# aokomoriuta/ConjugateGradient

Measured on AMD Instinct MI355X. Metric: CG iterations/sec (7-pt Poisson 512^3); SpMV achieved HBM GB/s in roofline, higher is better.
Workload: dtype f64

## Files before the change

### conjugategradient_amd/csrc/common.hpp

```cpp
#pragma once
#include <hip/hip_runtime.h>
#include <cstddef>
#include <cstdint>
#include <cstdio>
#include <cstdarg>
#include <cstring>
#include <cmath>
#include <atomic>
#include <mutex>
#include <string>
#include <type_traits>
#include <vector>

#pragma GCC visibility push(default)
#include "../../include/MgcgGpu.h"
#pragma GCC visibility pop

namespace mgcg {

constexpr int kWave = 64;
constexpr int kBlock = 256;
constexpr int kNumXcd = 8;
constexpr int kNumCu = 256;
constexpr int kMaxGrid = kNumCu * 8;
// ... 379 lines not shown
struct SpmvConfig { int kernel = 0; int rowsPerBlock = 64; int flags = 0; int gridBlocks = 0; int periodRows = 0; int tileRows = 0; int tilePlanes = 0;
                    int maxRow = 0;  };

int launch_spmv(hipStream_t s, int epilogue, const SpmvArgs& a, const SpmvConfig& cfg);
inline bool spmv_takes_rowtile(const SpmvArgs& a, const SpmvConfig& cfg)
{
    int kernel = cfg.kernel;
    if (kernel == 0) kernel = spmv_auto_kernel(a.rowCount > 0 ? (double)a.elementsCount / (double)a.rowCount : 0.0);
    return kernel == 10 && (((uintptr_t)a.elements & 15) == 0) && (((uintptr_t)a.columnIndeces & 15) == 0) && a.elementsCount >= 8 && a.rowCount > 0;
}
int launch_spmv_rowtile(hipStream_t s, int epilogue, const SpmvArgs& a, int periodRows, int gridReq, int maxRow = 0, bool ntWindow = false,
                        int gapAtTile = 0, int gapSkipTiles = 0);
int spmv_period(MgcgSparse* h, const int* rowOffsets, const int* columnIndeces, long long rows, long long rowBase, int* maxRow = nullptr, long long* meanDistance = nullptr);
void launch_matrix_shape(hipStream_t s, const int* rowOffsets, const int* columnIndeces, long long rows, long long row, long long rowBase, int* out2);
int launch_spmv_rows(hipStream_t s, int epilogue, const SpmvArgs& a, const DcsrView* m, int gridReq, int periodRows = 0);
bool dcsr_build(hipStream_t s, const double* elements, const int* rowOffsets, const int* columnIndeces,
                long long rows, long long nnz, long long rowBase, DcsrMatrix* out);
bool pattern_build(hipStream_t s, const double* elements, const int* rowOffsets, const int* columnIndeces,
                   long long rows, long long nnz, long long rowBase, DcsrMatrix* out);
bool tiled_build(hipStream_t s, const double* elements, const int* rowOffsets, const int* columnIndeces,
                 long long rows, long long nnz, long long rowBase, long long columns, DcsrMatrix* out);
int launch_spmv_tiled(hipStream_t s, int epilogue, const SpmvArgs& a, const DcsrView& m);
bool exclusive_scan(hipStream_t s, int* data, long long n);
bool pb_build(hipStream_t s, const double* elements, const int* rowOffsets, const int* columnIndeces,
              long long rows, long long nnz, long long columns, long long meanDistance, DcsrMatrix* out);
int launch_spmv_pb(hipStream_t s, int epilogue, const SpmvArgs& a, const DcsrView& m);
const DcsrMatrix* dcsr_lookup(MgcgSparse* h, const double* elements, const int* rowOffsets, const int* columnIndeces,
                              long long rows, long long nnz, long long rowBase, long long columns = 0,
                              long long autoMeanDistance = -1,
                              bool trustRegistry = false);
const DcsrMatrix* dcsr_lookup_op(MgcgSparse* h, const SpmvArgs& a, long long rowBase);
bool vector_owned(const void* p, size_t bytes);
void vector_registry_add(const void* p, size_t bytes);
void vector_registry_remove(const void* p);
unsigned long long csr_checksum(hipStream_t s, const double* elements, const int* rowOffsets, const int* columnIndeces, long long rows, long long nnz, unsigned long long* scratch);
void analysis_note_write(const void* p, size_t bytes);
int launch_spmv_auto(hipStream_t s, int epilogue, const SpmvArgs& a, const SpmvConfig& cfg, const DcsrMatrix* dc);
int launch_spmv_range(hipStream_t s, int epilogue, const SpmvArgs& a, const SpmvConfig& cfg, const DcsrMatrix* dc,
                      long long r0, long long r1, double* partials, int maxGrid);

int launch_spmv_two_ranges(hipStream_t s, int epilogue, const SpmvArgs& a, const SpmvConfig& cfg, const DcsrMatrix* dc,
                           long long i0, long long i1, double* partials, int maxGrid);

void launch_axpy(hipStream_t s, double* y, const double* x, long long n, double alpha);
void launch_scal(hipStream_t s, double* x, double alpha, long long n);
void launch_xpay(hipStream_t s, double* y, const double* x, long long n, double beta);
// ... 189 lines not shown
    default:                 converged = (it >= f.minIt) && (it <= f.maxIt) && (d.res < f.tol); break;
    }
    d.status = MGCG_OK;
    d.stop = converged;
    if (!d.stop && it >= f.minIt && it > f.maxIt) { d.stop = true; d.status = MGCG_MAXIT_EXCEEDED; }
    if (!d.stop && !(d.res == d.res && fabs(d.res) <= 1.79e308)) { d.stop = true; d.status = MGCG_NONFINITE; }
    return d;
}
void launch_reduce_to(hipStream_t s, const double* partials, int n, double* dst, const int* done);
void launch_reduce2_to(hipStream_t s, const double* pA, int nA, double* dstA, const double* pB, int nB, double* dstB, const int* done);
void launch_finalize(hipStream_t s, const double* partials, const double* partialsInf, int n, bool reduceFirst, const FinalizeArgs& f);
void launch_finalize_precond(hipStream_t s, const double* partials, int n, bool reduceFirst, CgScalars* sc);
void launch_init_scalars(hipStream_t s, const double* partials, const double* partialsZ, int n, bool reduceFirst, CgScalars* sc, HostMirror* mirror);

void launch_jacobi_first(hipStream_t s, long long n, double omega, const double* dinv, int dinvUniform, double dinvScalar, const double* b, double* x, const int* done);
void launch_uniform_check(hipStream_t s, const double* v, long long n, int* flag);
void launch_restrict(hipStream_t s, int nx, int ny, int nz, const double* r, double* bc, const int* done);
void launch_prolong_add(hipStream_t s, int nx, int ny, int nz, double* x, const double* e, const int* done);
void launch_prolong_linear_add(hipStream_t s, int nx, int ny, int nz, int z0, int z1, double* x, const double* eFull, const int* done);
void launch_restrict_linear(hipStream_t s, int nx, int ny, int nz, int z0, int z1, const double* rFull, double* bc, const int* done);
void launch_prolong_scaled(hipStream_t s, int nx, int ny, int nz, double* x, const double* b, double inner, double outer, const double* e, const int* done);
void launch_extract_dinv(hipStream_t s, const double* elements, const int* rowOffsets, const int* columnIndeces,
                         long long n, long long rowBase, double* dinv);
void launch_galerkin(hipStream_t s, int nx, int ny, int nz, int zBegin, int zEnd, const double* elements, const int* rowOffsets, const int* columnIndeces,
                     double sigma, const int* rowOffsetsC, int* countsC, double* elementsC, int* columnIndecesC, int* errFlag);
void launch_poisson(hipStream_t s, int nx, int ny, int nz, int zBegin, int zEnd, double* elements, int* rowOffsets, int* columnIndeces);
void launch_rebase(hipStream_t s, int* rowOffsets, long long n, int base);
long long poisson_nnz_host(int nx, int ny, int nz, int zBegin, int zEnd);
void launch_minmax_int(hipStream_t s, const int* v, long long n, int* out2 );
void launch_halo_rows(hipStream_t s, const int* rowOffsets, const int* columnIndeces, long long n, long long offset, int* out2 );

void launch_amg_restrict(hipStream_t s, long long nc, const int* aggOffsets, const int* members, const double* r, double* bc, const int* done);
void launch_amg_prolong_add(hipStream_t s, long long n, const int* agg, double* x, const double* e, const int* done);
void launch_amg_check_diagonal(hipStream_t s, const double* elements, const int* rowOffsets, const int* columnIndeces, long long n, int* badRow);
void launch_amg_row_max(hipStream_t s, const double* elements, const int* rowOffsets, const int* columnIndeces, long long n, double* rowMax);
void launch_amg_match_round(hipStream_t s, const double* elements, const int* rowOffsets, const int* columnIndeces, long long n, double theta,
                            const double* rowMax, int* match, int* pick, int* flags2);
void launch_amg_galerkin_count(hipStream_t s, long long nc, const int* aggOffsets, const int* members, const int* rowOffsets, const int* columnIndeces,
                               const int* agg, const int* expandOffsets, int* scratch, int* counts);
void launch_amg_galerkin_fill(hipStream_t s, long long nc, const int* aggOffsets, const int* members, const double* elements, const int* rowOffsets,
                              const int* columnIndeces, const int* agg, const int* expandOffsets, const int* scratch, const int* rowOffsetsC, double sigma,
                              double* elementsC, int* columnIndecesC);
void launch_amg_gather_values(hipStream_t s, long long m, const int* source, const double* elements, double* out);

constexpr int kTransposeShortMax = 32;
constexpr int kTransposeLdsMax = 4096;
void launch_transpose_check_offsets(hipStream_t s, const int* rowOffsets, long long rows, int* status3);
void launch_transpose_count(hipStream_t s, const int* rowOffsets, const int* columnIndeces, long long rows, long long columns, long long nnz, int* counts, int* badRow);
// ... 47 lines not shown
```

### conjugategradient_amd/csrc/kernels_mg.hip

```cpp
#include "common.hpp"

namespace mgcg {

static inline int grid1(long long n)
{
    long long b = (n + kBlock - 1) / kBlock;
    if (b > kMaxGrid) b = kMaxGrid;
    if (b < 1) b = 1;
    return (int)b;
}

typedef double d2mg __attribute__((ext_vector_type(2)));

template <bool UNIFORM>
__global__ __launch_bounds__(kBlock) void jacobi_first_kernel(long long n, double omega, const double* __restrict__ dinv, double dscalar,
                                                              const double* __restrict__ b, double* __restrict__ x, const int* done)
{
    if (done != nullptr && *done != 0) return;
    const bool wide = ((((uintptr_t)b) | ((uintptr_t)x) | ((uintptr_t)dinv)) & 15) == 0;
    if (wide) {
        const long long n2 = n >> 1;
        const long long per = ((n2 + gridDim.x - 1) / gridDim.x + (kBlock - 1)) & ~(long long)(kBlock - 1);
        long long end = per * (blockIdx.x + 1);
        end = end < n2 ? end : n2;
// ... 323 lines not shown
        return;
    }
    const long long NC = (long long)(nx > 1 ? nx / 2 : 1) * (ny > 1 ? ny / 2 : 1) * ((z1 - z0) / (nz > 1 ? 2 : 1));
    hipLaunchKernelGGL(restrict_linear_kernel, dim3(grid1(NC)), dim3(kBlock), 0, s, nx, ny, nz, z0, z1, rFull, bc, done);
}

__global__ __launch_bounds__(kBlock) void extract_dinv_kernel(const double* __restrict__ elements, const int* __restrict__ rowOffsets,
                                                              const int* __restrict__ columnIndeces, long long n, long long rowBase, double* __restrict__ dinv)
{
    const long long stride = (long long)gridDim.x * kBlock;
    for (long long i = (long long)blockIdx.x * kBlock + threadIdx.x; i < n; i += stride) {
        double d = 0.0;
        for (int k = rowOffsets[i]; k < rowOffsets[i + 1]; ++k)
            if (columnIndeces[k] == rowBase + i) { d = elements[k]; break; }
        dinv[i] = 1.0 / d;
    }
}
void launch_extract_dinv(hipStream_t s, const double* elements, const int* rowOffsets, const int* columnIndeces,
                         long long n, long long rowBase, double* dinv)
{
    hipLaunchKernelGGL(extract_dinv_kernel, dim3(grid1(n)), dim3(kBlock), 0, s, elements, rowOffsets, columnIndeces, n, rowBase, dinv);
}

__global__ __launch_bounds__(kBlock) void galerkin_kernel(int nx, int ny, int nz, int zBegin, int zEnd,
                                                          const double* __restrict__ elements, const int* __restrict__ rowOffsets,
                                                          const int* __restrict__ columnIndeces, double sigma, const int* __restrict__ rowOffsetsC,
                                                          int* __restrict__ countsC, double* __restrict__ elementsC, int* __restrict__ columnIndecesC, int* errFlag)
{
    const int cx = nx > 1 ? 2 : 1, cy = ny > 1 ? 2 : 1, cz = nz > 1 ? 2 : 1;
    const int NX = nx / cx, NY = ny / cy;
    const int ZL = (zEnd - zBegin) / cz;
    const int Z0 = zBegin / cz;
    const long long NC = (long long)NX * NY * ZL;
    const long long sxy = (long long)nx * ny;
    const long long stride = (long long)gridDim.x * kBlock;
    for (long long I = (long long)blockIdx.x * kBlock + threadIdx.x; I < NC; I += stride) {
        const int X = (int)(I % NX), Y = (int)((I / NX) % NY), Zl = (int)(I / ((long long)NX * NY));
        const int Z = Z0 + Zl;
        double acc[27];
        unsigned touched = 0u;
#pragma unroll
        for (int q = 0; q < 27; ++q) acc[q] = 0.0;
        for (int dz = 0; dz < cz; ++dz)
            for (int dy = 0; dy < cy; ++dy)
                for (int dx = 0; dx < cx; ++dx) {
                    const long long i = ((long long)(Zl * cz + dz) * ny + (Y * cy + dy)) * nx + (X * cx + dx);
                    for (int k = rowOffsets[i]; k < rowOffsets[i + 1]; ++k) {
                        const long long j = columnIndeces[k];
                        const int jx = (int)(j % nx), jy = (int)((j / nx) % ny), jz = (int)(j / sxy);
                        const int ox = jx / cx - X, oy = jy / cy - Y, oz = jz / cz - Z;
                        if (ox < -1 || ox > 1 || oy < -1 || oy > 1 || oz < -1 || oz > 1) { *errFlag = 1; continue; }
                        const int q = (oz + 1) * 9 + (oy + 1) * 3 + (ox + 1);
                        const double v = elements[k];
#pragma unroll
                        for (int t = 0; t < 27; ++t) if (t == q) acc[t] += v;
                        touched |= 1u << q;
                    }
                }
        if (elementsC == nullptr) { countsC[I] = __popc(touched); continue; }
        int kout = rowOffsetsC[I];
#pragma unroll
        for (int q = 0; q < 27; ++q) {
            if (!(touched & (1u << q))) continue;
            const int ox = q % 3 - 1, oy = (q / 3) % 3 - 1, oz = q / 9 - 1;
            elementsC[kout] = sigma * acc[q];
            columnIndecesC[kout] = (int)(((long long)(Z + oz) * NY + (Y + oy)) * NX + (X + ox));
            ++kout;
        }
    }
}
void launch_galerkin(hipStream_t s, int nx, int ny, int nz, int zBegin, int zEnd, const double* elements, const int* rowOffsets, const int* columnIndeces,
                     double sigma, const int* rowOffsetsC, int* countsC, double* elementsC, int* columnIndecesC, int* errFlag)
{
    const long long NC = (long long)(nx > 1 ? nx / 2 : 1) * (ny > 1 ? ny / 2 : 1) * (nz > 1 ? (zEnd - zBegin) / 2 : 1);
    hipLaunchKernelGGL(galerkin_kernel, dim3(grid1(NC)), dim3(kBlock), 0, s, nx, ny, nz, zBegin, zEnd, elements, rowOffsets, columnIndeces,
                       sigma, rowOffsetsC, countsC, elementsC, columnIndecesC, errFlag);
}

__device__ __host__ inline long long poisson_row_offset(long long i, int nx, int ny, int nz)
{
    const long long sxy = (long long)nx * ny;
    const int x = (int)(i % nx), y = (int)((i / nx) % ny), z = (int)(i / sxy);
    const long long L = i / nx;
    long long missing = 0;
    missing += L + (x > 0 ? 1 : 0);
    missing += L;
    missing += (long long)z * nx + (y > 0 ? nx : x);
    missing += (long long)z * nx + (y == ny - 1 ? x : 0);
    if (nz > 1) {
        missing += (z > 0) ? sxy : ((long long)y * nx + x);
        missing += (z == nz - 1) ? ((long long)y * nx + x) : 0;
        return 7 * i - missing;
    }
    return 5 * i - missing;
}

__global__ __launch_bounds__(kBlock) void poisson_kernel(int nx, int ny, int nz, int zBegin, int zEnd,
                                                         double* __restrict__ elements, int* __restrict__ rowOffsets, int* __restrict__ columnIndeces)
{
// ... 103 lines not shown
```

### conjugategradient_amd/csrc/kernels_tiled.hip

```cpp
#include "common.hpp"
#include <algorithm>

namespace mgcg {

constexpr int kScanBlock = 256;
constexpr int kScanPer = 8;

__global__ __launch_bounds__(kBlock) void tiled_count_kernel(const int* __restrict__ rowOffsets, const int* __restrict__ columnIndeces,
                                                             long long rows, long long rowBase, int tileWidth, int nTiles,
                                                             int* __restrict__ counts, unsigned long long* stats )
{
    const long long stride = (long long)gridDim.x * kBlock;
    unsigned long long far = 0, unsorted = 0;
    for (long long i = (long long)blockIdx.x * kBlock + threadIdx.x; i < rows; i += stride) {
        const int s = rowOffsets[i], e = rowOffsets[i + 1];
        int prev = -1, tile = -1, run = 0;
        for (int k = s; k < e; ++k) {
            const int c = columnIndeces[k];
            if (c <= prev) unsorted = 1;
            prev = c;
            const long long d = (long long)c - (rowBase + i);
            far += (unsigned long long)((d < 0 ? -d : d) >> 10);
            const int t = c / tileWidth;
            if (t != tile) { if (tile >= 0 && tile < nTiles) counts[(long long)tile * rows + i] = run; tile = t; run = 0; }
// ... 5 lines not shown
    if (unsorted) atomicAdd(&stats[0], 1ull);
}

__global__ __launch_bounds__(kScanBlock) void scan_local_kernel(int* __restrict__ data, long long n, int* __restrict__ blockTotals)
{
    __shared__ int s_sum[kScanBlock];
    const long long base = ((long long)blockIdx.x * kScanBlock + threadIdx.x) * kScanPer;
    int v[kScanPer], total = 0;
#pragma unroll
    for (int j = 0; j < kScanPer; ++j) { v[j] = (base + j < n) ? data[base + j] : 0; total += v[j]; }
    s_sum[threadIdx.x] = total;
    __syncthreads();
    for (int off = 1; off < kScanBlock; off <<= 1) {
        const int add = threadIdx.x >= off ? s_sum[threadIdx.x - off] : 0;
        __syncthreads();
        s_sum[threadIdx.x] += add;
        __syncthreads();
    }
    int run = s_sum[threadIdx.x] - total;
#pragma unroll
    for (int j = 0; j < kScanPer; ++j) { if (base + j < n) data[base + j] = run; run += v[j]; }
    if (threadIdx.x == kScanBlock - 1) blockTotals[blockIdx.x] = s_sum[kScanBlock - 1];
}
__global__ __launch_bounds__(kScanBlock) void scan_totals_kernel(int* __restrict__ blockTotals, int nBlocks)
{
    __shared__ int s_sum[kScanBlock];
    __shared__ int s_carry;
    if (threadIdx.x == 0) s_carry = 0;
    __syncthreads();
    for (int base = 0; base < nBlocks; base += kScanBlock) {
        const int i = base + threadIdx.x;
        const int v = i < nBlocks ? blockTotals[i] : 0;
        s_sum[threadIdx.x] = v;
        __syncthreads();
        for (int off = 1; off < kScanBlock; off <<= 1) {
            const int add = threadIdx.x >= off ? s_sum[threadIdx.x - off] : 0;
            __syncthreads();
            s_sum[threadIdx.x] += add;
            __syncthreads();
        }
        if (i < nBlocks) blockTotals[i] = s_carry + s_sum[threadIdx.x] - v;
        __syncthreads();
        if (threadIdx.x == kScanBlock - 1) s_carry += s_sum[kScanBlock - 1];
        __syncthreads();
    }
}
__global__ __launch_bounds__(kScanBlock) void scan_add_kernel(int* __restrict__ data, long long n, const int* __restrict__ blockTotals)
{
    const long long base = ((long long)blockIdx.x * kScanBlock + threadIdx.x) * kScanPer;
    const int add = blockTotals[blockIdx.x];
#pragma unroll
    for (int j = 0; j < kScanPer; ++j) if (base + j < n) data[base + j] += add;
}

__global__ __launch_bounds__(kBlock) void tiled_zero_kernel(double* __restrict__ y, long long n, const int* __restrict__ doneFlag)
{
    if (doneFlag != nullptr && *doneFlag != 0) return;
    const long long stride = (long long)gridDim.x * kBlock;
    for (long long i = (long long)blockIdx.x * kBlock + threadIdx.x; i < n; i += stride) y[i] = 0.0;
}
static int grid_rows(long long n)
{
    const long long blocks = (n + kBlock - 1) / kBlock;
    return (int)(blocks < 1 ? 1 : (blocks > kMaxGrid ? kMaxGrid : blocks));
}

__global__ __launch_bounds__(kBlock) void tiled_scatter_kernel(const double* __restrict__ elements, const int* __restrict__ rowOffsets,
                                                               const int* __restrict__ columnIndeces, long long rows, int tileWidth,
// ... 179 lines not shown
        hipLaunchKernelGGL(spmv_tile_pass_kernel<false>, g, dim3(kBlock), 0, s, a.x, a.y, m.tileVals, m.tileCols, m.tileRowIds, kb, ke, a.doneFlag);
    }
    if (EPI == EPI_AXPBY && a.alpha == 1.0) return 0;
    const int grid = grid_rows(a.rowCount);
    hipLaunchKernelGGL((tiled_epilogue_kernel<EPI>), dim3(grid), dim3(kBlock), 0, s, a);
    return grid;
}

int launch_spmv_tiled(hipStream_t s, int epilogue, const SpmvArgs& a, const DcsrView& m)
{
    if (a.rowCount <= 0) return 0;
    switch (epilogue) {
    case EPI_AXPBY:        return launch_tiled_epi<EPI_AXPBY>(s, a, m);
    case EPI_DOT:          return launch_tiled_epi<EPI_DOT>(s, a, m);
    case EPI_RESIDUAL:     return launch_tiled_epi<EPI_RESIDUAL>(s, a, m);
    case EPI_RESIDUAL_DOT: return launch_tiled_epi<EPI_RESIDUAL_DOT>(s, a, m);
    case EPI_JACOBI:       return launch_tiled_epi<EPI_JACOBI>(s, a, m);
    case EPI_JACOBI_DOT:   return launch_tiled_epi<EPI_JACOBI_DOT>(s, a, m);
    }
    set_error("column-tiled SpMV: epilogue %d is not implemented (the Chebyshev step multiplies through the CSR kernels)", epilogue);
    return 0;
}

bool exclusive_scan(hipStream_t s, int* data, long long n)
{
    const long long perBlock = (long long)kScanBlock * kScanPer;
    const long long nBlocks = (n + perBlock - 1) / perBlock;
    if (nBlocks > 0x7fffffffLL) { set_error("tiled analysis: too many scan blocks"); return false; }
    int* totals = nullptr;
    if (!MGCG_HIP(hipMalloc((void**)&totals, sizeof(int) * (size_t)nBlocks))) return false;
    hipLaunchKernelGGL(scan_local_kernel, dim3((unsigned)nBlocks), dim3(kScanBlock), 0, s, data, n, totals);
    hipLaunchKernelGGL(scan_totals_kernel, dim3(1), dim3(kScanBlock), 0, s, totals, (int)nBlocks);
    hipLaunchKernelGGL(scan_add_kernel, dim3((unsigned)nBlocks), dim3(kScanBlock), 0, s, data, n, totals);
    const bool ok = MGCG_HIP(hipGetLastError()) && MGCG_HIP(hipStreamSynchronize(s));
    (void)hipFree(totals);
    return ok;
}

bool tiled_build(hipStream_t s, const double* elements, const int* rowOffsets, const int* columnIndeces,
                 long long rows, long long nnz, long long rowBase, long long columns, DcsrMatrix* out)
{
    int tileShift = 19;
    long long tileCols = 365LL * 1024;
    { const int v = tuning().tileShift.load(std::memory_order_relaxed); if (v >= 8 && v <= 26) { tileShift = v; tileCols = 1LL << v; } }
    const int nTiles = (int)((columns + tileCols - 1) / tileCols);
    const int tileWidth = nTiles > 0 ? (int)((columns + nTiles - 1) / nTiles) : (int)tileCols;
    if (rows <= 0 || nnz <= 0 || nTiles < 4 || nTiles > 256) return true;
    const long long cells = (long long)nTiles * rows;
    {
        size_t freeB = 0, totalB = 0;
        if (hipMemGetInfo(&freeB, &totalB) != hipSuccess) { (void)hipGetLastError(); return true; }
        const double need = 4.0 * (double)(cells + 1) + 16.0 * (double)nnz;
        if (cells + 1 > 0x7fffffffLL * 4LL || need > 0.5 * (double)freeB) return true;
    }
    int* counts = nullptr; unsigned long long* stats = nullptr;
    double* tv = nullptr; int* tc = nullptr; int* tr = nullptr;
// ... 88 lines not shown
```

### conjugategradient_amd/csrc/solver.hip

```cpp
#include "common.hpp"
#include <algorithm>
#include <chrono>
#include <functional>

namespace mgcg {

struct MgLevel {
    int nx = 0, ny = 0, nz = 0;
    int z0 = 0, z1 = 0;
    long long n = 0, nnz = 0;
    long long nGlobal = 0, offset = 0;
    double* elements = nullptr; int* rowOffsets = nullptr; int* columnIndeces = nullptr;
    bool ownsMatrix = false;
    double* dinv = nullptr;
    bool dinvUniform = false; double dinvScalar = 0.0;
    double *xa = nullptr, *xb = nullptr;
    double *b = nullptr, *r = nullptr;
    SpmvConfig cfg;
    const DcsrMatrix* dcsr = nullptr;
    HaloPlan* halo = nullptr;
    HaloPlan* transferHalo = nullptr;
    int minJ = 0, maxJ = -1;
    bool overlap = false;
    long long interior0 = 0, interior1 = 0;
// ... 2003 lines not shown
                        int elementsCount, int nx, int ny, int nz, int zBegin, int zEnd,
                        int levels, double omega, int nu, int nuCoarse, double sigma)
{
    DeviceState* d = device_state();
    if (!d) return nullptr;
    const long long nGlobal0 = (long long)nx * ny * nz;
    const int nranks = MgcgCommSize(comm);
    const long long nLocal0 = (long long)nx * ny * (zEnd - zBegin);
    bool pre = true;
    if (!cublas || !cusparse || !elementsVector || !rowOffsetsVector || !columnIndecesVector) { set_error("MgSetup: null argument"); pre = false; }
    if (pre && (nx < 1 || ny < 1 || nz < 1 || levels < 1 || nu < 1 || nuCoarse < 1 || nGlobal0 > 0x7fffffffLL || zBegin < 0 || zEnd > nz || zBegin >= zEnd)) { set_error("MgSetup: bad parameters"); pre = false; }
    if (pre && (rowOffsetsVector->size < nLocal0 + 1 || elementsVector->size < elementsCount || columnIndecesVector->size < elementsCount)) { set_error("MgSetup: matrix vectors too small"); pre = false; }
    if (pre && nranks > 1 && (nz % nranks != 0 || (zEnd - zBegin) != nz / nranks || zBegin != MgcgCommRank(comm) * (nz / nranks))) {
        set_error("MgSetup: with several ranks the grid must be split into equal z-slabs in rank order"); pre = false;
    }
    if (!comm_agree(comm, pre, "MgSetup")) return nullptr;
    hipStream_t s = d->stream;
    MgcgMg* mg = new MgcgMg();
    mg->omega = omega; mg->nu = nu; mg->nuCoarse = nuCoarse; mg->sigma = sigma; mg->stream = s; mg->cfg = cfg_of(cusparse);
    mg->cfg.kernel = 0;
    mg->comm = comm; mg->nranks = nranks; mg->multi = comm_multi(comm);
    mg->haloOnSide = tuning().haloStream.load(std::memory_order_relaxed) != 0;
    const bool multi = mg->multi;
    int* dErr = nullptr;
    int* dmm = nullptr;
    bool ok = MGCG_HIP(hipMalloc((void**)&dErr, sizeof(int))) && MGCG_HIP(hipMemsetAsync(dErr, 0, sizeof(int), s)) && MGCG_HIP(hipMalloc((void**)&dmm, 2 * sizeof(int)));
    auto coarse_matrix = [&](MgLevel& L, const MgLevel& F) -> bool {
        L.ownsMatrix = true;
        int* counts = nullptr;
        bool good = MGCG_HIP(hipMalloc((void**)&L.rowOffsets, sizeof(int) * (size_t)(L.n + 1))) && MGCG_HIP(hipMalloc((void**)&counts, sizeof(int) * (size_t)(L.n > 0 ? L.n : 1)));
        std::vector<int> h((size_t)L.n + 1);
        int err = 0;
        if (good) {
            launch_galerkin(s, F.nx, F.ny, F.nz, F.z0, F.z1, F.elements, F.rowOffsets, F.columnIndeces, sigma, nullptr, counts, nullptr, nullptr, dErr);
            good = MGCG_HIP(hipMemcpyAsync(h.data() + 1, counts, sizeof(int) * (size_t)L.n, hipMemcpyDeviceToHost, s)) &&
                   MGCG_HIP(hipMemcpyAsync(&err, dErr, sizeof(int), hipMemcpyDeviceToHost, s)) && MGCG_HIP(hipStreamSynchronize(s));
        }
        if (counts) (void)hipFree(counts);
        if (!good) return false;
        if (err) { set_error("MgSetup: matrix is not a 27-point-neighbourhood operator on the %dx%dx%d grid", F.nx, F.ny, F.nz); return false; }
        h[0] = 0;
        long long run = 0;
        for (long long i = 1; i <= L.n; ++i) { run += h[(size_t)i]; h[(size_t)i] = (int)run; }
        L.nnz = run;
        good = MGCG_HIP(hipMemcpyAsync(L.rowOffsets, h.data(), sizeof(int) * (size_t)(L.n + 1), hipMemcpyHostToDevice, s)) &&
               MGCG_HIP(hipMalloc((void**)&L.elements, sizeof(double) * (size_t)(L.nnz > 0 ? L.nnz : 1))) &&
               MGCG_HIP(hipMalloc((void**)&L.columnIndeces, sizeof(int) * (size_t)(L.nnz > 0 ? L.nnz : 1)));
        if (good) launch_galerkin(s, F.nx, F.ny, F.nz, F.z0, F.z1, F.elements, F.rowOffsets, F.columnIndeces, sigma, L.rowOffsets, nullptr, L.elements, L.columnIndeces, dErr);
        return MGCG_HIP(hipStreamSynchronize(s)) && good;
    };
    bool agreedToLeave = false;
    for (int l = 0; ok && l < levels; ++l) {
        MgLevel L;
        if (l == 0) {
            L.nx = nx; L.ny = ny; L.nz = nz; L.z0 = zBegin; L.z1 = zEnd; L.nnz = elementsCount;
            L.elements = elementsVector->data; L.rowOffsets = rowOffsetsVector->data; L.columnIndeces = columnIndecesVector->data;
        } else {
            const MgLevel& F = mg->lv[l - 1];
            if ((F.nx > 1 && F.nx % 2) || (F.ny > 1 && F.ny % 2) || (F.nz > 1 && F.nz % 2)) break;
            if (F.nx == 1 && F.ny == 1 && F.nz == 1) break;
            if (F.nz > 1 && ((F.z0 % 2) || (F.z1 % 2))) break;
            if (nranks > 1 && F.nz == 1) break;
            L.nx = F.nx > 1 ? F.nx / 2 : 1; L.ny = F.ny > 1 ? F.ny / 2 : 1; L.nz = F.nz > 1 ? F.nz / 2 : 1;
            L.z0 = F.nz > 1 ? F.z0 / 2 : 0; L.z1 = F.nz > 1 ? F.z1 / 2 : 1;
        }
        L.nGlobal = (long long)L.nx * L.ny * L.nz;
        L.n = (long long)L.nx * L.ny * (L.z1 - L.z0);
        L.offset = (long long)L.nx * L.ny * L.z0;
        if (l > 0) ok = ok && coarse_matrix(L, mg->lv[l - 1]);
        ok = ok && MGCG_HIP(hipMalloc((void**)&L.dinv, sizeof(double) * (size_t)L.n));
        ok = ok && MGCG_HIP(hipMalloc((void**)&L.xa, sizeof(double) * (size_t)L.nGlobal));
        ok = ok && MGCG_HIP(hipMalloc((void**)&L.r, sizeof(double) * (size_t)L.n));
        if (l > 0 || multi) ok = ok && MGCG_HIP(hipMalloc((void**)&L.xb, sizeof(double) * (size_t)L.nGlobal));
        if (l > 0) ok = ok && MGCG_HIP(hipMalloc((void**)&L.b, sizeof(double) * (size_t)L.n));
        if (ok && multi) {
            ok = ok && MGCG_HIP(hipMemsetAsync(L.xa, 0, sizeof(double) * (size_t)L.nGlobal, s)) && MGCG_HIP(hipMemsetAsync(L.xb, 0, sizeof(double) * (size_t)L.nGlobal, s));
        }
        if (ok) launch_extract_dinv(s, L.elements, L.rowOffsets, L.columnIndeces, L.n, L.offset, L.dinv);
        if (ok && L.n > 0) {
            int differs = 1;
            ok = MGCG_HIP(hipMemsetAsync(dmm, 0, sizeof(int), s));
            if (ok) launch_uniform_check(s, L.dinv, L.n, dmm);
            ok = ok && MGCG_HIP(hipMemcpyAsync(&differs, dmm, sizeof(int), hipMemcpyDeviceToHost, s)) &&
                 MGCG_HIP(hipMemcpyAsync(&L.dinvScalar, L.dinv, sizeof(double), hipMemcpyDeviceToHost, s)) && MGCG_HIP(hipStreamSynchronize(s));
            L.dinvUniform = ok && differs == 0;
        }
        if (ok) L.dcsr = dcsr_lookup(cusparse, L.elements, L.rowOffsets, L.columnIndeces, L.n, L.nnz, L.offset);
        L.cfg = mg->cfg;
        if (ok && L.nnz >= 8) (void)spmv_period(cusparse, L.rowOffsets, L.columnIndeces, L.n, L.offset, &L.cfg.maxRow);
        L.cfg.periodRows = (L.nz > 1) ? L.nx * L.ny : 0;
        if (ok && multi) {
            int init[2] = { 0x7fffffff, (int)0x80000000 }, out[2] = { 0, -1 };
            ok = ok && MGCG_HIP(hipMemcpyAsync(dmm, init, sizeof(init), hipMemcpyHostToDevice, s));
            if (ok && L.nnz > 0) launch_minmax_int(s, L.columnIndeces, L.nnz, dmm);
            ok = ok && MGCG_HIP(hipMemcpyAsync(out, dmm, sizeof(out), hipMemcpyDeviceToHost, s));
            ok = ok && MGCG_HIP(hipStreamSynchronize(s));
            L.minJ = out[0]; L.maxJ = out[1];
        }
        if (multi) {
            ok = comm_agree(comm, ok, "MgSetup");
            if (ok) { L.halo = halo_plan_create(comm, L.nGlobal, L.offset, L.n, L.minJ, L.maxJ); ok = comm_agree(comm, L.halo != nullptr, "MgSetup"); }
            agreedToLeave = !ok;
            ok = ok && plan_overlap(s, comm, mg->multi, L.rowOffsets, L.columnIndeces, L.n, L.offset, &L.overlap, &L.interior0, &L.interior1, cublas->ws.devInts + 6, L.halo, L.xa, L.nGlobal);
        }
        mg->lv.push_back(L);
        if (!ok) break;
        mg->levels = (int)mg->lv.size();
    }
    ok = ok && MGCG_HIP(hipStreamSynchronize(s));
    if (dErr) (void)hipFree(dErr);
    if (dmm) (void)hipFree(dmm);
    bool wantDeep = ok && multi && nu == 1 && mg->levels >= 2 && tuning().deepHalo.load(std::memory_order_relaxed) != 0;
    bool foldsEverywhere = true;
    for (int l = 1; wantDeep && l < mg->levels; ++l) {
        const MgLevel& L = mg->lv[(size_t)l];
        const int d = (l == mg->levels - 1) ? nuCoarse : 2;
        if (L.nz <= 1 || (L.z1 - L.z0) < d || (L.z0 & 1) || ((L.z1 - L.z0) & 1)) wantDeep = false;
    }
    if (multi && (agreedToLeave || !comm_agree(comm, ok, "MgSetup"))) { MgDestroy(mg); return nullptr; }
    for (int l = 1; ok && wantDeep && l < mg->levels; ++l) {
        MgLevel& L = mg->lv[(size_t)l];
        const long long plane = (long long)L.nx * L.ny;
        const int d = (l == mg->levels - 1) ? nuCoarse : 2;
        L.deep = d;
        L.extZ0 = L.z0 - d < 0 ? 0 : L.z0 - d;
        L.extZ1 = L.z1 + d > L.nz ? L.nz : L.z1 + d;
        L.extBase = (long long)L.extZ0 * plane; L.extRows = (long long)(L.extZ1 - L.extZ0) * plane;
        const long long edge = (long long)d * plane;
        std::vector<int> ro((size_t)L.n + 1);
        bool lok = MGCG_HIP(hipMemcpyAsync(ro.data(), L.rowOffsets, sizeof(int) * (size_t)(L.n + 1), hipMemcpyDeviceToHost, s)) && MGCG_HIP(hipStreamSynchronize(s));
        auto pack = [&](long long r0, long long r1, std::vector<double>& out) {
            out.clear();
            if (!lok || r1 <= r0) return;
// ... 1450 lines not shown
```

Baseline: 275.6.

## Tile Galerkin coarsening in LDS, scan row offsets on device, fuse dinv extraction

Rewrites the Galerkin coarse-operator kernel to stage row offsets, column indices and values for a tile of 64 coarse rows in shared memory. It replaces integer division with magic-number reciprocals and splits the 27 stencil slots across four lanes per coarse row. The host-side prefix sum and its round trip are replaced by a device exclusive scan. The coarse diagonal inverse and its uniformity check are computed inside the fill kernel, which removes the separate extract and check passes and several stream syncs. All of this is MG setup work, so the timed CG/SpMV iteration throughput is unlikely to change.

```diff
diff --git a/conjugategradient_amd/csrc/common.hpp b/conjugategradient_amd/csrc/common.hpp
--- a/conjugategradient_amd/csrc/common.hpp
+++ b/conjugategradient_amd/csrc/common.hpp
@@ -425,6 +425,8 @@
                  long long rows, long long nnz, long long rowBase, long long columns, DcsrMatrix* out);
 int launch_spmv_tiled(hipStream_t s, int epilogue, const SpmvArgs& a, const DcsrView& m);
 bool exclusive_scan(hipStream_t s, int* data, long long n);
+long long exclusive_scan_blocks(long long n);
+void exclusive_scan_enqueue(hipStream_t s, int* data, long long n, int* totals, int* totalOut);
 bool pb_build(hipStream_t s, const double* elements, const int* rowOffsets, const int* columnIndeces,
               long long rows, long long nnz, long long columns, long long meanDistance, DcsrMatrix* out);
 int launch_spmv_pb(hipStream_t s, int epilogue, const SpmvArgs& a, const DcsrView& m);
@@ -660,8 +662,15 @@
 void launch_prolong_scaled(hipStream_t s, int nx, int ny, int nz, double* x, const double* b, double inner, double outer, const double* e, const int* done);
 void launch_extract_dinv(hipStream_t s, const double* elements, const int* rowOffsets, const int* columnIndeces,
                          long long n, long long rowBase, double* dinv);
+struct MgSetupRecord {
+    int nnz;
+    int err;
+    unsigned long long dinvHi;
+    unsigned long long dinvLo;
+    double dinvFirst;
+};
 void launch_galerkin(hipStream_t s, int nx, int ny, int nz, int zBegin, int zEnd, const double* elements, const int* rowOffsets, const int* columnIndeces,
-                     double sigma, const int* rowOffsetsC, int* countsC, double* elementsC, int* columnIndecesC, int* errFlag);
+                     long long nnzF, double sigma, const int* rowOffsetsC, int* countsC, double* elementsC, int* columnIndecesC, double* dinvC, MgSetupRecord* rec);
 void launch_poisson(hipStream_t s, int nx, int ny, int nz, int zBegin, int zEnd, double* elements, int* rowOffsets, int* columnIndeces);
 void launch_rebase(hipStream_t s, int* rowOffsets, long long n, int base);
 long long poisson_nnz_host(int nx, int ny, int nz, int zBegin, int zEnd);
diff --git a/conjugategradient_amd/csrc/kernels_mg.hip b/conjugategradient_amd/csrc/kernels_mg.hip
--- a/conjugategradient_amd/csrc/kernels_mg.hip
+++ b/conjugategradient_amd/csrc/kernels_mg.hip
@@ -369,59 +369,234 @@
     hipLaunchKernelGGL(extract_dinv_kernel, dim3(grid1(n)), dim3(kBlock), 0, s, elements, rowOffsets, columnIndeces, n, rowBase, dinv);
 }
 
+typedef int i4mg __attribute__((ext_vector_type(4)));
+constexpr int kGalTile = 64;
+constexpr int kGalRuns = 4;
+constexpr int kGalCap = kGalRuns * 2 * kGalTile * 7 + 8 * kGalRuns;
+static_assert(kBlock == 4 * kGalTile, "four lanes per coarse row of a tile");
+
+struct GalDiv { unsigned long long m; int shift; };
+__device__ __forceinline__ GalDiv gal_div(unsigned d)
+{
+    const int l = d > 1u ? 32 - __clz((int)(d - 1u)) : 0;
+    return { ((1ull << (31 + l)) + d - 1u) / d, 31 + l };
+}
+__device__ __forceinline__ unsigned gal_quot(unsigned n, GalDiv g) { return (unsigned)(((unsigned long long)n * g.m) >> g.shift); }
+
+struct GalGrid { unsigned nx, sxy; GalDiv byLine, byPlane; int sx, sy, sz; };
+__device__ __forceinline__ int gal_slot(const GalGrid& g, int col, int X, int Y, int Z)
+{
+    if (col < 0) return -1;
+    const unsigned j = (unsigned)col;
+    const unsigned jz = gal_quot(j, g.byPlane), rem = j - jz * g.sxy, jy = gal_quot(rem, g.byLine), jx = rem - jy * g.nx;
+    const int ox = (int)(jx >> g.sx) - X, oy = (int)(jy >> g.sy) - Y, oz = (int)(jz >> g.sz) - Z;
+    if (ox < -1 || ox > 1 || oy < -1 || oy > 1 || oz < -1 || oz > 1) return -1;
+    return (oz + 1) * 9 + (oy + 1) * 3 + (ox + 1);
+}
+
+template <bool FILL>
 __global__ __launch_bounds__(kBlock) void galerkin_kernel(int nx, int ny, int nz, int zBegin, int zEnd,
                                                           const double* __restrict__ elements, const int* __restrict__ rowOffsets,
-                                                          const int* __restrict__ columnIndeces, double sigma, const int* __restrict__ rowOffsetsC,
-                                                          int* __restrict__ countsC, double* __restrict__ elementsC, int* __restrict__ columnIndecesC, int* errFlag)
-{
+                                                          const int* __restrict__ columnIndeces, long long nnzF, double sigma,
+                                                          const int* __restrict__ rowOffsetsC, int* __restrict__ countsC, double* __restrict__ elementsC,
+                                                          int* __restrict__ columnIndecesC, double* __restrict__ dinvC, MgSetupRecord* rec)
+{
+    __shared__ int s_ro[kGalRuns][2 * kGalTile + 1];
+    __shared__ __attribute__((aligned(16))) int s_col[kGalCap];
+    __shared__ __attribute__((aligned(16))) double s_val[FILL ? kGalCap : 2];
+    __shared__ unsigned s_touched[kGalTile];
+    __shared__ unsigned long long s_hi, s_lo;
     const int cx = nx > 1 ? 2 : 1, cy = ny > 1 ? 2 : 1, cz = nz > 1 ? 2 : 1;
     const int NX = nx / cx, NY = ny / cy;
     const int ZL = (zEnd - zBegin) / cz;
     const int Z0 = zBegin / cz;
-    const long long NC = (long long)NX * NY * ZL;
-    const long long sxy = (long long)nx * ny;
-    const long long stride = (long long)gridDim.x * kBlock;
-    for (long long I = (long long)blockIdx.x * kBlock + threadIdx.x; I < NC; I += stride) {
-        const int X = (int)(I % NX), Y = (int)((I / NX) % NY), Zl = (int)(I / ((long long)NX * NY));
+    const int runs = cy * cz;
+    const int tilesX = (NX + kGalTile - 1) / kGalTile;
+    const long long nTiles = (long long)tilesX * NY * ZL;
+    GalGrid grid;
+    grid.nx = (unsigned)nx; grid.sxy = (unsigned)nx * (unsigned)ny;
+    grid.byLine = gal_div(grid.nx); grid.byPlane = gal_div(grid.sxy);
+    grid.sx = cx - 1; grid.sy = cy - 1; grid.sz = cz - 1;
+    const bool aligned = ((((uintptr_t)elements) | ((uintptr_t)columnIndeces)) & 15) == 0;
+    const int mine = (int)threadIdx.x & (kGalTile - 1), part = (int)threadIdx.x / kGalTile;
+    unsigned long long hi = 0ull, lo = 0ull;
+    if (threadIdx.x == 0) { s_hi = 0ull; s_lo = 0ull; }
+    for (long long tile = blockIdx.x; tile < nTiles; tile += gridDim.x) {
+        const int X0 = (int)(tile % tilesX) * kGalTile;
+        const long long line = tile / tilesX;
+        const int Y = (int)(line % NY), Zl = (int)(line / NY);
         const int Z = Z0 + Zl;
-        double acc[27];
-        unsigned touched = 0u;
-#pragma unroll
-        for (int q = 0; q < 27; ++q) acc[q] = 0.0;
-        for (int dz = 0; dz < cz; ++dz)
-            for (int dy = 0; dy < cy; ++dy)
+        const long long I0 = ((long long)Zl * NY + Y) * NX + X0;
+        const int rowsC = NX - X0 < kGalTile ? NX - X0 : kGalTile;
+        const int rowsF = rowsC * cx;
+        for (int t = threadIdx.x; t < runs * (rowsF + 1); t += kBlock) {
+            const int r = t / (rowsF + 1), f = t - r * (rowsF + 1);
+            const int dz = r / cy, dy = r - dz * cy;
+            const long long i0 = ((long long)(Zl * cz + dz) * ny + (Y * cy + dy)) * nx + X0 * cx;
+            s_ro[r][f] = rowOffsets[i0 + f];
+        }
+        if (!FILL && threadIdx.x < kGalTile) s_touched[threadIdx.x] = 0u;
+        __syncthreads();
+        int a0[kGalRuns], a1[kGalRuns], base[kGalRuns];
+        int total = 0;
+        bool sane = true;
+#pragma unroll
+        for (int r = 0; r < kGalRuns; ++r) {
+            a0[r] = 0; a1[r] = 0; base[r] = total;
+            if (r < runs) {
+                a0[r] = s_ro[r][0] & ~3;
+                a1[r] = (s_ro[r][rowsF] + 3) & ~3;
+                sane = sane && s_ro[r][0] >= 0 && a1[r] >= a0[r] && a1[r] - a0[r] <= kGalCap;
+                total += a1[r] - a0[r];
+            }
+        }
+        const bool parked = aligned && sane && total <= kGalCap;
+        if (parked) {
+#pragma unroll
+            for (int r = 0; r < kGalRuns; ++r) {
+                const int groups = (a1[r] - a0[r]) >> 2;
+                for (int g = threadIdx.x; g < groups; g += kBlock) {
+                    const long long k = (long long)a0[r] + 4 * g;
+                    const int at = base[r] + 4 * g;
+                    if (k + 4 <= nnzF) {
+                        *(i4mg*)&s_col[at] = *(const i4mg*)&columnIndeces[k];
+                        if (FILL) {
+                            *(d2mg*)&s_val[at] = *(const d2mg*)&elements[k];
+                            *(d2mg*)&s_val[at + 2] = *(const d2mg*)&elements[k + 2];
+                        }
+                    } else {
+                        for (int j = 0; j < 4; ++j)
+                            if (k + j < nnzF) { s_col[at + j] = columnIndeces[k + j]; if (FILL) s_val[at + j] = elements[k + j]; }
+                    }
+                }
+            }
+            __syncthreads();
+            for (int t = threadIdx.x; t < runs * rowsF; t += kBlock) {
+                const int r = t / rowsF, f = t - r * rowsF;
+                const int shift = r == 0 ? base[0] - a0[0] : r == 1 ? base[1] - a0[1] : r == 2 ? base[2] - a0[2] : base[3] - a0[3];
+                const int c = f >> grid.sx;
+                unsigned slots = 0u;
+                const int kEnd = s_ro[r][f + 1];
+                for (int k = s_ro[r][f]; k < kEnd; ++k) {
+                    const int q = gal_slot(grid, s_col[k + shift], X0 + c, Y, Z);
+                    if (q < 0) rec->err = 1; else slots |= 1u << q;
+                    if (FILL) s_col[k + shift] = q;
+                }
+                if (!FILL && slots != 0u) atomicOr(&s_touched[c], slots);
+            }
+            __syncthreads();
+            if (!FILL) {
+                if ((int)threadIdx.x < rowsC) countsC[I0 + threadIdx.x] = __popc(s_touched[threadIdx.x]);
+            } else if (mine < rowsC) {
+                const long long I = I0 + mine;
+                const int X = X0 + mine;
+                double acc[7];
+                unsigned touched = 0u;
+#pragma unroll
+                for (int t = 0; t < 7; ++t) acc[t] = 0.0;
+#pragma unroll
+                for (int r = 0; r < kGalRuns; ++r) {
+                    if (r >= runs) break;
+                    const int shift = base[r] - a0[r];
+                    for (int dx = 0; dx < cx; ++dx) {
+                        const int f = mine * cx + dx;
+                        const int kEnd = s_ro[r][f + 1];
+                        for (int k = s_ro[r][f]; k < kEnd; ++k) {
+                            const int q = s_col[k + shift];
+                            if (q < 0) continue;
+                            touched |= 1u << q;
+                            if ((q & 3) != part) continue;
+                            const double v = s_val[k + shift];
+                            const int at = q >> 2;
+#pragma unroll
+                            for (int t = 0; t < 7; ++t) if (t == at) acc[t] += v;
+                        }
+                    }
+                }
+                const int kbase = rowOffsetsC[I];
+#pragma unroll
+                for (int t = 0; t < 7; ++t) {
+                    const int q = 4 * t + part;
+                    if (q >= 27 || !(touched & (1u << q))) continue;
+                    const int kout = kbase + __popc(touched & ((1u << q) - 1u));
+                    const int ox = q % 3 - 1, oy = (q / 3) % 3 - 1, oz = q / 9 - 1;
+                    elementsC[kout] = sigma * acc[t];
+                    columnIndecesC[kout] = (int)(((long long)(Z + oz) * NY + (Y + oy)) * NX + (X + ox));
+                }
+                if (part == 1) {
+                    const double d = (touched & (1u << 13)) ? sigma * acc[3] : 0.0;
+                    const double di = 1.0 / d;
+                    dinvC[I] = di;
+                    const unsigned long long bits = (unsigned long long)__double_as_longlong(di);
+                    hi = bits > hi ? bits : hi;
+                    lo = ~bits > lo ? ~bits : lo;
+                    if (I == 0) rec->dinvFirst = di;
+                }
+            }
+        } else if ((int)threadIdx.x < rowsC) {
+            const long long I = I0 + threadIdx.x;
+            const int X = X0 + (int)threadIdx.x;
+            double acc[27];
+            unsigned touched = 0u;
+#pragma unroll
+            for (int q = 0; q < 27; ++q) acc[q] = 0.0;
+            for (int r = 0; r < runs; ++r)
                 for (int dx = 0; dx < cx; ++dx) {
-                    const long long i = ((long long)(Zl * cz + dz) * ny + (Y * cy + dy)) * nx + (X * cx + dx);
-                    for (int k = rowOffsets[i]; k < rowOffsets[i + 1]; ++k) {
-                        const long long j = columnIndeces[k];
-                        const int jx = (int)(j % nx), jy = (int)((j / nx) % ny), jz = (int)(j / sxy);
-                        const int ox = jx / cx - X, oy = jy / cy - Y, oz = jz / cz - Z;
-                        if (ox < -1 || ox > 1 || oy < -1 || oy > 1 || oz < -1 || oz > 1) { *errFlag = 1; continue; }
-                        const int q = (oz + 1) * 9 + (oy + 1) * 3 + (ox + 1);
-                        const double v = elements[k];
-#pragma unroll
-                        for (int t = 0; t < 27; ++t) if (t == q) acc[t] += v;
+                    const int f = (int)threadIdx.x * cx + dx;
+                    const int kEnd = s_ro[r][f + 1];
+                    for (int k = s_ro[r][f]; k < kEnd; ++k) {
+                        const int q = gal_slot(grid, columnIndeces[k], X, Y, Z);
+                        if (q < 0) { rec->err = 1; continue; }
+                        if (FILL) {
+                            const double v = elements[k];
+#pragma unroll
+                            for (int t = 0; t < 27; ++t) if (t == q) acc[t] += v;
+                        }
                         touched |= 1u << q;
                     }
                 }
-        if (elementsC == nullptr) { countsC[I] = __popc(touched); continue; }
-        int kout = rowOffsetsC[I];
-#pragma unroll
-        for (int q = 0; q < 27; ++q) {
-            if (!(touched & (1u << q))) continue;
-            const int ox = q % 3 - 1, oy = (q / 3) % 3 - 1, oz = q / 9 - 1;
-            elementsC[kout] = sigma * acc[q];
-            columnIndecesC[kout] = (int)(((long long)(Z + oz) * NY + (Y + oy)) * NX + (X + ox));
-            ++kout;
-        }
+            if (!FILL) countsC[I] = __popc(touched);
+            else {
+                int kout = rowOffsetsC[I];
+#pragma unroll
+                for (int q = 0; q < 27; ++q) {
+                    if (!(touched & (1u << q))) continue;
+                    const int ox = q % 3 - 1, oy = (q / 3) % 3 - 1, oz = q / 9 - 1;
+                    elementsC[kout] = sigma * acc[q];
+                    columnIndecesC[kout] = (int)(((long long)(Z + oz) * NY + (Y + oy)) * NX + (X + ox));
+                    ++kout;
+                }
+                const double d = (touched & (1u << 13)) ? sigma * acc[13] : 0.0;
+                const double di = 1.0 / d;
+                dinvC[I] = di;
+                const unsigned long long bits = (unsigned long long)__double_as_longlong(di);
+                hi = bits > hi ? bits : hi;
+                lo = ~bits > lo ? ~bits : lo;
+                if (I == 0) rec->dinvFirst = di;
+            }
+        }
+        __syncthreads();
+    }
+    if (FILL) {
+        atomicMax(&s_hi, hi);
+        atomicMax(&s_lo, lo);
+        __syncthreads();
+        if (threadIdx.x == 0) { atomicMax(&rec->dinvHi, s_hi); atomicMax(&rec->dinvLo, s_lo); }
     }
 }
 void launch_galerkin(hipStream_t s, int nx, int ny, int nz, int zBegin, int zEnd, const double* elements, const int* rowOffsets, const int* columnIndeces,
-                     double sigma, const int* rowOffsetsC, int* countsC, double* elementsC, int* columnIndecesC, int* errFlag)
-{
-    const long long NC = (long long)(nx > 1 ? nx / 2 : 1) * (ny > 1 ? ny / 2 : 1) * (nz > 1 ? (zEnd - zBegin) / 2 : 1);
-    hipLaunchKernelGGL(galerkin_kernel, dim3(grid1(NC)), dim3(kBlock), 0, s, nx, ny, nz, zBegin, zEnd, elements, rowOffsets, columnIndeces,
-                       sigma, rowOffsetsC, countsC, elementsC, columnIndecesC, errFlag);
+                     long long nnzF, double sigma, const int* rowOffsetsC, int* countsC, double* elementsC, int* columnIndecesC, double* dinvC, MgSetupRecord* rec)
+{
+    const int NX = nx > 1 ? nx / 2 : 1;
+    const long long nTiles = (long long)((NX + kGalTile - 1) / kGalTile) * (ny > 1 ? ny / 2 : 1) * (nz > 1 ? (zEnd - zBegin) / 2 : 1);
+    if (nTiles <= 0) return;
+    const int grid = (int)(nTiles > kMaxGrid ? kMaxGrid : nTiles);
+    if (elementsC == nullptr)
+        hipLaunchKernelGGL(galerkin_kernel<false>, dim3(grid), dim3(kBlock), 0, s, nx, ny, nz, zBegin, zEnd, elements, rowOffsets, columnIndeces,
+                           nnzF, sigma, rowOffsetsC, countsC, elementsC, columnIndecesC, dinvC, rec);
+    else
+        hipLaunchKernelGGL(galerkin_kernel<true>, dim3(grid), dim3(kBlock), 0, s, nx, ny, nz, zBegin, zEnd, elements, rowOffsets, columnIndeces,
+                           nnzF, sigma, rowOffsetsC, countsC, elementsC, columnIndecesC, dinvC, rec);
 }
 
 __device__ __host__ inline long long poisson_row_offset(long long i, int nx, int ny, int nz)
diff --git a/conjugategradient_amd/csrc/kernels_tiled.hip b/conjugategradient_amd/csrc/kernels_tiled.hip
--- a/conjugategradient_amd/csrc/kernels_tiled.hip
+++ b/conjugategradient_amd/csrc/kernels_tiled.hip
@@ -51,7 +51,7 @@
     for (int j = 0; j < kScanPer; ++j) { if (base + j < n) data[base + j] = run; run += v[j]; }
     if (threadIdx.x == kScanBlock - 1) blockTotals[blockIdx.x] = s_sum[kScanBlock - 1];
 }
-__global__ __launch_bounds__(kScanBlock) void scan_totals_kernel(int* __restrict__ blockTotals, int nBlocks)
+__global__ __launch_bounds__(kScanBlock) void scan_totals_kernel(int* __restrict__ blockTotals, int nBlocks, int* __restrict__ totalOut)
 {
     __shared__ int s_sum[kScanBlock];
     __shared__ int s_carry;
@@ -73,6 +73,7 @@
         if (threadIdx.x == kScanBlock - 1) s_carry += s_sum[kScanBlock - 1];
         __syncthreads();
     }
+    if (totalOut != nullptr && threadIdx.x == 0) *totalOut = s_carry;
 }
 __global__ __launch_bounds__(kScanBlock) void scan_add_kernel(int* __restrict__ data, long long n, const int* __restrict__ blockTotals)
 {
@@ -298,16 +299,26 @@
     return 0;
 }
 
+long long exclusive_scan_blocks(long long n)
+{
+    const long long perBlock = (long long)kScanBlock * kScanPer;
+    return (n + perBlock - 1) / perBlock;
+}
+void exclusive_scan_enqueue(hipStream_t s, int* data, long long n, int* totals, int* totalOut)
+{
+    const long long nBlocks = exclusive_scan_blocks(n);
+    if (nBlocks < 1) return;
+    hipLaunchKernelGGL(scan_local_kernel, dim3((unsigned)nBlocks), dim3(kScanBlock), 0, s, data, n, totals);
+    hipLaunchKernelGGL(scan_totals_kernel, dim3(1), dim3(kScanBlock), 0, s, totals, (int)nBlocks, totalOut);
+    hipLaunchKernelGGL(scan_add_kernel, dim3((unsigned)nBlocks), dim3(kScanBlock), 0, s, data, n, totals);
+}
 bool exclusive_scan(hipStream_t s, int* data, long long n)
 {
-    const long long perBlock = (long long)kScanBlock * kScanPer;
-    const long long nBlocks = (n + perBlock - 1) / perBlock;
+    const long long nBlocks = exclusive_scan_blocks(n);
     if (nBlocks > 0x7fffffffLL) { set_error("tiled analysis: too many scan blocks"); return false; }
     int* totals = nullptr;
     if (!MGCG_HIP(hipMalloc((void**)&totals, sizeof(int) * (size_t)nBlocks))) return false;
-    hipLaunchKernelGGL(scan_local_kernel, dim3((unsigned)nBlocks), dim3(kScanBlock), 0, s, data, n, totals);
-    hipLaunchKernelGGL(scan_totals_kernel, dim3(1), dim3(kScanBlock), 0, s, totals, (int)nBlocks);
-    hipLaunchKernelGGL(scan_add_kernel, dim3((unsigned)nBlocks), dim3(kScanBlock), 0, s, data, n, totals);
+    exclusive_scan_enqueue(s, data, n, totals, nullptr);
     const bool ok = MGCG_HIP(hipGetLastError()) && MGCG_HIP(hipStreamSynchronize(s));
     (void)hipFree(totals);
     return ok;
diff --git a/conjugategradient_amd/csrc/solver.hip b/conjugategradient_amd/csrc/solver.hip
--- a/conjugategradient_amd/csrc/solver.hip
+++ b/conjugategradient_amd/csrc/solver.hip
@@ -2049,32 +2049,44 @@
     mg->comm = comm; mg->nranks = nranks; mg->multi = comm_multi(comm);
     mg->haloOnSide = tuning().haloStream.load(std::memory_order_relaxed) != 0;
     const bool multi = mg->multi;
-    int* dErr = nullptr;
     int* dmm = nullptr;
-    bool ok = MGCG_HIP(hipMalloc((void**)&dErr, sizeof(int))) && MGCG_HIP(hipMemsetAsync(dErr, 0, sizeof(int), s)) && MGCG_HIP(hipMalloc((void**)&dmm, 2 * sizeof(int)));
-    auto coarse_matrix = [&](MgLevel& L, const MgLevel& F) -> bool {
+    MgSetupRecord* dRec = nullptr;
+    std::vector<MgSetupRecord> hRec((size_t)levels);
+    bool ok = MGCG_HIP(hipMalloc((void**)&dRec, sizeof(MgSetupRecord) * (size_t)levels)) && MGCG_HIP(hipMemsetAsync(dRec, 0, sizeof(MgSetupRecord) * (size_t)levels, s)) &&
+              MGCG_HIP(hipMalloc((void**)&dmm, 2 * sizeof(int)));
+    int verdictDue = -1;
+    auto take_verdict = [&](int l) {
+        MgLevel& V = mg->lv[(size_t)l];
+        V.dinvUniform = hRec[(size_t)l].dinvHi == ~hRec[(size_t)l].dinvLo;
+        V.dinvScalar = hRec[(size_t)l].dinvFirst;
+    };
+    auto coarse_matrix = [&](int l, MgLevel& L, const MgLevel& F) -> bool {
         L.ownsMatrix = true;
-        int* counts = nullptr;
-        bool good = MGCG_HIP(hipMalloc((void**)&L.rowOffsets, sizeof(int) * (size_t)(L.n + 1))) && MGCG_HIP(hipMalloc((void**)&counts, sizeof(int) * (size_t)(L.n > 0 ? L.n : 1)));
-        std::vector<int> h((size_t)L.n + 1);
-        int err = 0;
+        int* totals = nullptr;
+        MgSetupRecord* rec = dRec + l;
+        bool good = MGCG_HIP(hipMalloc((void**)&L.rowOffsets, sizeof(int) * (size_t)(L.n + 1))) && MGCG_HIP(hipMalloc((void**)&totals, sizeof(int) * (size_t)exclusive_scan_blocks(L.n + 1))) &&
+                    MGCG_HIP(hipMemsetAsync(L.rowOffsets + L.n, 0, sizeof(int), s));
         if (good) {
-            launch_galerkin(s, F.nx, F.ny, F.nz, F.z0, F.z1, F.elements, F.rowOffsets, F.columnIndeces, sigma, nullptr, counts, nullptr, nullptr, dErr);
-            good = MGCG_HIP(hipMemcpyAsync(h.data() + 1, counts, sizeof(int) * (size_t)L.n, hipMemcpyDeviceToHost, s)) &&
-                   MGCG_HIP(hipMemcpyAsync(&err, dErr, sizeof(int), hipMemcpyDeviceToHost, s)) && MGCG_HIP(hipStreamSynchronize(s));
-        }
-        if (counts) (void)hipFree(counts);
+            launch_galerkin(s, F.nx, F.ny, F.nz, F.z0, F.z1, F.elements, F.rowOffsets, F.columnIndeces, F.nnz, sigma, nullptr, L.rowOffsets, nullptr, nullptr, nullptr, rec);
+            exclusive_scan_enqueue(s, L.rowOffsets, L.n + 1, totals, &rec->nnz);
+            const int first = verdictDue >= 0 ? verdictDue : l;
+            good = MGCG_HIP(hipGetLastError()) && MGCG_HIP(hipMemcpyAsync(&hRec[(size_t)first], dRec + first, sizeof(MgSetupRecord) * (size_t)(l - first + 1), hipMemcpyDeviceToHost, s)) &&
+                   MGCG_HIP(hipStreamSynchronize(s));
+        }
+        if (totals) (void)hipFree(totals);
         if (!good) return false;
-        if (err) { set_error("MgSetup: matrix is not a 27-point-neighbourhood operator on the %dx%dx%d grid", F.nx, F.ny, F.nz); return false; }
-        h[0] = 0;
-        long long run = 0;
-        for (long long i = 1; i <= L.n; ++i) { run += h[(size_t)i]; h[(size_t)i] = (int)run; }
-        L.nnz = run;
-        good = MGCG_HIP(hipMemcpyAsync(L.rowOffsets, h.data(), sizeof(int) * (size_t)(L.n + 1), hipMemcpyHostToDevice, s)) &&
-               MGCG_HIP(hipMalloc((void**)&L.elements, sizeof(double) * (size_t)(L.nnz > 0 ? L.nnz : 1))) &&
-               MGCG_HIP(hipMalloc((void**)&L.columnIndeces, sizeof(int) * (size_t)(L.nnz > 0 ? L.nnz : 1)));
-        if (good) launch_galerkin(s, F.nx, F.ny, F.nz, F.z0, F.z1, F.elements, F.rowOffsets, F.columnIndeces, sigma, L.rowOffsets, nullptr, L.elements, L.columnIndeces, dErr);
-        return MGCG_HIP(hipStreamSynchronize(s)) && good;
+        if (verdictDue >= 0) { take_verdict(verdictDue); verdictDue = -1; }
+        if (hRec[(size_t)l].err) { set_error("MgSetup: matrix is not a 27-point-neighbourhood operator on the %dx%dx%d grid", F.nx, F.ny, F.nz); return false; }
+        L.nnz = hRec[(size_t)l].nnz;
+        good = MGCG_HIP(hipMalloc((void**)&L.elements, sizeof(double) * (size_t)(L.nnz > 0 ? L.nnz : 1))) &&
+               MGCG_HIP(hipMalloc((void**)&L.columnIndeces, sizeof(int) * (size_t)(L.nnz > 0 ? L.nnz : 1))) &&
+               MGCG_HIP(hipMalloc((void**)&L.dinv, sizeof(double) * (size_t)L.n));
+        if (good) {
+            launch_galerkin(s, F.nx, F.ny, F.nz, F.z0, F.z1, F.elements, F.rowOffsets, F.columnIndeces, F.nnz, sigma, L.rowOffsets, nullptr, L.elements, L.columnIndeces, L.dinv, rec);
+            good = MGCG_HIP(hipGetLastError());
+            verdictDue = l;
+        }
+        return good;
     };
     bool agreedToLeave = false;
     for (int l = 0; ok && l < levels; ++l) {
@@ -2094,8 +2106,8 @@
         L.nGlobal = (long long)L.nx * L.ny * L.nz;
         L.n = (long long)L.nx * L.ny * (L.z1 - L.z0);
         L.offset = (long long)L.nx * L.ny * L.z0;
-        if (l > 0) ok = ok && coarse_matrix(L, mg->lv[l - 1]);
-        ok = ok && MGCG_HIP(hipMalloc((void**)&L.dinv, sizeof(double) * (size_t)L.n));
+        if (l > 0) ok = ok && coarse_matrix(l, L, mg->lv[l - 1]);
+        else ok = ok && MGCG_HIP(hipMalloc((void**)&L.dinv, sizeof(double) * (size_t)L.n));
         ok = ok && MGCG_HIP(hipMalloc((void**)&L.xa, sizeof(double) * (size_t)L.nGlobal));
         ok = ok && MGCG_HIP(hipMalloc((void**)&L.r, sizeof(double) * (size_t)L.n));
         if (l > 0 || multi) ok = ok && MGCG_HIP(hipMalloc((void**)&L.xb, sizeof(double) * (size_t)L.nGlobal));
@@ -2103,8 +2115,8 @@
         if (ok && multi) {
             ok = ok && MGCG_HIP(hipMemsetAsync(L.xa, 0, sizeof(double) * (size_t)L.nGlobal, s)) && MGCG_HIP(hipMemsetAsync(L.xb, 0, sizeof(double) * (size_t)L.nGlobal, s));
         }
-        if (ok) launch_extract_dinv(s, L.elements, L.rowOffsets, L.columnIndeces, L.n, L.offset, L.dinv);
-        if (ok && L.n > 0) {
+        if (ok && l == 0) launch_extract_dinv(s, L.elements, L.rowOffsets, L.columnIndeces, L.n, L.offset, L.dinv);
+        if (ok && l == 0 && L.n > 0) {
             int differs = 1;
             ok = MGCG_HIP(hipMemsetAsync(dmm, 0, sizeof(int), s));
             if (ok) launch_uniform_check(s, L.dinv, L.n, dmm);
@@ -2134,8 +2146,10 @@
         if (!ok) break;
         mg->levels = (int)mg->lv.size();
     }
+    if (ok && verdictDue >= 0) ok = MGCG_HIP(hipMemcpyAsync(&hRec[(size_t)verdictDue], dRec + verdictDue, sizeof(MgSetupRecord), hipMemcpyDeviceToHost, s));
     ok = ok && MGCG_HIP(hipStreamSynchronize(s));
-    if (dErr) (void)hipFree(dErr);
+    if (ok && verdictDue >= 0) take_verdict(verdictDue);
+    if (dRec) (void)hipFree(dRec);
     if (dmm) (void)hipFree(dmm);
     bool wantDeep = ok && multi && nu == 1 && mg->levels >= 2 && tuning().deepHalo.load(std::memory_order_relaxed) != 0;
     bool foldsEverywhere = true;
```

Measured after the change: 270.1. 0.98x the previous value.
